# Hjinhan/Transgo

Measured on AMD Instinct MI355X. Metric: MCTS simulations/sec, higher is better.
Workload: dtype f32

## Files before the change

### include/transgo_hip.h

```cpp
#ifndef TRANSGO_HIP_H_
#define TRANSGO_HIP_H_

#include <stdbool.h>
#include <stddef.h>
#include <stdint.h>

#ifdef __cplusplus
extern "C" {
#endif

typedef struct tg_ctx tg_ctx;

typedef enum tg_status {
    TG_OK = 0,
    TG_ERR_ARG = -1,
    TG_ERR_HIP = -2,
    TG_ERR_NO_DEVICE = -3,
    TG_ERR_ARENA = -4,
    TG_ERR_STATE = -5
} tg_status;

typedef struct tg_config {
    int32_t board_size;
    int32_t encode_dim;
// ... 65 lines not shown
int tg_sp_rng_get(tg_ctx* ctx, tg_mt19937* out );
int tg_sp_rng_set(tg_ctx* ctx, const tg_mt19937* in , const uint8_t* mask );
int tg_sp_play(tg_ctx* ctx, const int32_t* actions , uint8_t* done );
int tg_sp_game_errors(tg_ctx* ctx, int32_t* n_errors, int32_t* err );
int tg_sp_tree_truncations(tg_ctx* ctx, uint64_t* blocks);

int tg_sp_pool_stats(tg_ctx* ctx, uint64_t* pool_slots, uint64_t* high_water_slots, uint64_t* in_use_slots, uint64_t* exhausted);

int tg_sp_finished(tg_ctx* ctx, int32_t* n_games, int32_t* n_positions);
int tg_sp_harvest(tg_ctx* ctx, uint32_t* obs_bits, int32_t* counts, float* z, int8_t* own, uint8_t* player, int device_out,
                  int32_t* slot, int32_t* n_moves, int32_t* winner, float* score, int8_t* terr);
int tg_sp_final(tg_ctx* ctx, float* score , float* terr , int32_t* winner );
int tg_sp_stats(tg_ctx* ctx, uint64_t* sims, uint64_t* evals, uint64_t* depth_sum, uint64_t* tie_draws, int32_t* errors,
                int32_t* max_slots);

size_t tg_net_blob_floats(int board_size, int encode_dim, int filters, int blocks);
int tg_net_load(tg_ctx* ctx, const float* blob, size_t n_floats, int rows_cap);
size_t tg_net_blob_floats_arch(int board_size, int encode_dim, int filters, const char* arch);
int tg_net_load_arch(tg_ctx* ctx, const char* arch, const float* blob, size_t n_floats, int rows_cap);
int tg_net_load_async(tg_ctx* ctx, const char* arch, const float* blob, size_t n_floats);
int tg_net_load_async_dev(tg_ctx* ctx, const char* arch, const float* d_blob , size_t n_floats);
int tg_net_load_poll(tg_ctx* ctx, int wait, int* pending);
int tg_net_predict(tg_ctx* ctx, const float* obs, int n_rows, float* policy, float* value, float* own);
int tg_net_range(tg_ctx* ctx, uint64_t* fp16_overflows, float* weight_absmax);
int tg_prof_enable(tg_ctx* ctx, int on, int max_launches);
int tg_prof_read(tg_ctx* ctx, double* conv_ms, int64_t* conv_launches, double* conv_flops);
int tg_prof_skipped(tg_ctx* ctx, int64_t* launches);
int tg_prof_enable_tree(tg_ctx* ctx, int on, int max_waves);
int tg_prof_read_tree(tg_ctx* ctx, double* collect_ms, double* absorb_ms, int64_t* waves, uint64_t* children_scored);

typedef struct tg_replay tg_replay;
int tg_replay_create(tg_ctx* ctx, int capacity_positions, tg_replay** out);
void tg_replay_destroy(tg_replay* rp);
int tg_replay_append(tg_replay* rp, const uint32_t* obs_bits , const int32_t* counts ,
                     const float* z , const int8_t* own , int n);
int tg_replay_append_dev(tg_replay* rp, const uint32_t* obs_bits, const int32_t* counts, const float* z, const int8_t* own, int n);
int tg_replay_info(const tg_replay* rp, long long* entries, long long* index, int* full);
int tg_replay_sample(tg_replay* rp, const long long* entry , int B, float* state , float* pi ,
                     float* z , float* own , int device_out);


void tg_host_mt_seed(tg_mt19937* s, uint32_t seed);
uint32_t tg_host_mt_next32(tg_mt19937* s);
double tg_host_mt_random_sample(tg_mt19937* s);
int32_t tg_host_mt_choice_index(tg_mt19937* s, int32_t k);
int tg_host_mt_dirichlet(tg_mt19937* s, double alpha, int32_t n, double* out);
// ... 26 lines not shown
```

### transgo_amd/_lib.py

```python
import ctypes
import os

_HERE = os.path.dirname(os.path.abspath(__file__))
LIB_PATH = os.path.join(_HERE, "libtransgo_hip.so")


class TgConfig(ctypes.Structure):
    _fields_ = [("board_size", ctypes.c_int32), ("encode_dim", ctypes.c_int32), ("max_step", ctypes.c_int32),
                ("komi", ctypes.c_float), ("n_games", ctypes.c_int32), ("num_simulation", ctypes.c_int32),
                ("parallel_readouts", ctypes.c_int32), ("wu_loss", ctypes.c_int32), ("c_puct1", ctypes.c_double),
                ("c_puct2", ctypes.c_double), ("arena_slots", ctypes.c_int32), ("net_blocks", ctypes.c_int32),
                ("net_filters", ctypes.c_int32), ("device", ctypes.c_int32), ("net_precision", ctypes.c_int32),
                ("record_games", ctypes.c_int32), ("pool_slots", ctypes.c_int32), ("reserved", ctypes.c_int32 * 5)]


class TgMt19937(ctypes.Structure):
    _fields_ = [("key", ctypes.c_uint32 * 624), ("pos", ctypes.c_int32)]


class TransgoError(RuntimeError):
    pass


_lib = None
# ... 25 lines not shown
    "tg_sp_search": (ctypes.c_int, [_vp, ctypes.POINTER(ctypes.c_int32)]),
    "tg_sp_root_info": (ctypes.c_int, [_vp, _vp, _vp, _vp, _vp, _vp]),
    "tg_sp_draw_uniform": (ctypes.c_int, [_vp, _vp, _vp]),
    "tg_sp_rng_state": (ctypes.c_int, [_vp, ctypes.c_int, ctypes.POINTER(TgMt19937)]),
    "tg_sp_rng_get": (ctypes.c_int, [_vp, _vp]),
    "tg_sp_rng_set": (ctypes.c_int, [_vp, _vp, _vp]),
    "tg_sp_play": (ctypes.c_int, [_vp, _vp, _vp]),
    "tg_sp_final": (ctypes.c_int, [_vp, _vp, _vp, _vp]),
    "tg_sp_game_errors": (ctypes.c_int, [_vp, ctypes.POINTER(ctypes.c_int32), _vp]),
    "tg_sp_tree_truncations": (ctypes.c_int, [_vp, ctypes.POINTER(ctypes.c_uint64)]),
    "tg_sp_pool_stats": (ctypes.c_int, [_vp] + [ctypes.POINTER(ctypes.c_uint64)] * 4),
    "tg_sp_finished": (ctypes.c_int, [_vp, ctypes.POINTER(ctypes.c_int32), ctypes.POINTER(ctypes.c_int32)]),
    "tg_sp_harvest": (ctypes.c_int, [_vp, _vp, _vp, _vp, _vp, _vp, ctypes.c_int, _vp, _vp, _vp, _vp, _vp]),
    "tg_sp_stats": (ctypes.c_int, [_vp] + [ctypes.POINTER(ctypes.c_uint64)] * 4 + [ctypes.POINTER(ctypes.c_int32)] * 2),
    "tg_net_blob_floats": (ctypes.c_size_t, [ctypes.c_int] * 4),
    "tg_net_load": (ctypes.c_int, [_vp, _vp, ctypes.c_size_t, ctypes.c_int]),
    "tg_net_blob_floats_arch": (ctypes.c_size_t, [ctypes.c_int] * 3 + [ctypes.c_char_p]),
    "tg_net_load_arch": (ctypes.c_int, [_vp, ctypes.c_char_p, _vp, ctypes.c_size_t, ctypes.c_int]),
    "tg_net_load_async": (ctypes.c_int, [_vp, ctypes.c_char_p, _vp, ctypes.c_size_t]),
    "tg_net_load_async_dev": (ctypes.c_int, [_vp, ctypes.c_char_p, _vp, ctypes.c_size_t]),
    "tg_net_load_poll": (ctypes.c_int, [_vp, ctypes.c_int, ctypes.POINTER(ctypes.c_int)]),
    "tg_net_predict": (ctypes.c_int, [_vp, _vp, ctypes.c_int, _vp, _vp, _vp]),
    "tg_net_range": (ctypes.c_int, [_vp, ctypes.POINTER(ctypes.c_uint64), ctypes.POINTER(ctypes.c_float)]),
    "tg_prof_enable": (ctypes.c_int, [_vp, ctypes.c_int, ctypes.c_int]),
    "tg_prof_read": (ctypes.c_int, [_vp, ctypes.POINTER(ctypes.c_double), ctypes.POINTER(ctypes.c_int64), ctypes.POINTER(ctypes.c_double)]),
    "tg_prof_skipped": (ctypes.c_int, [_vp, ctypes.POINTER(ctypes.c_int64)]),
    "tg_prof_enable_tree": (ctypes.c_int, [_vp, ctypes.c_int, ctypes.c_int]),
    "tg_prof_read_tree": (ctypes.c_int, [_vp, ctypes.POINTER(ctypes.c_double), ctypes.POINTER(ctypes.c_double), ctypes.POINTER(ctypes.c_int64),
                                          ctypes.POINTER(ctypes.c_uint64)]),
    "tg_replay_create": (ctypes.c_int, [_vp, ctypes.c_int, ctypes.POINTER(ctypes.c_void_p)]),
    "tg_replay_destroy": (None, [_vp]),
    "tg_replay_append": (ctypes.c_int, [_vp, _vp, _vp, _vp, _vp, ctypes.c_int]),
    "tg_replay_append_dev": (ctypes.c_int, [_vp, _vp, _vp, _vp, _vp, ctypes.c_int]),
    "tg_replay_info": (ctypes.c_int, [_vp, ctypes.POINTER(ctypes.c_longlong), ctypes.POINTER(ctypes.c_longlong), ctypes.POINTER(ctypes.c_int)]),
    "tg_replay_sample": (ctypes.c_int, [_vp, _vp, ctypes.c_int, _vp, _vp, _vp, _vp, ctypes.c_int]),
    "tg_host_mt_seed": (None, [ctypes.POINTER(TgMt19937), ctypes.c_uint32]),
    "tg_host_mt_next32": (ctypes.c_uint32, [ctypes.POINTER(TgMt19937)]),
    "tg_host_mt_random_sample": (ctypes.c_double, [ctypes.POINTER(TgMt19937)]),
    "tg_host_mt_choice_index": (ctypes.c_int32, [ctypes.POINTER(TgMt19937), ctypes.c_int32]),
    "tg_host_sub_encode": (None, [ctypes.c_int, _vp, _vp, ctypes.c_int, ctypes.c_int, ctypes.c_int]),
    "tg_host_mt_dirichlet": (ctypes.c_int, [ctypes.POINTER(TgMt19937), ctypes.c_double, ctypes.c_int32, _vp]),
}


def load():
    global _lib
# ... 57 lines not shown
```

### transgo_amd/csrc/net.hip

```cpp
#include <cmath>
#include <cstdlib>
#include <cstring>
#include <string>
#include <vector>

#include "conv_rows.h"
#include "engine.h"

using namespace tg;

namespace tg {

struct ConvW { const float* w; const float* b; };
struct BlockW { const float* s1; const float* t1; ConvW c1; ConvW c2; const float* g1; const float* g2;
                const _Float16* h1; const _Float16* h2; };
struct AttW { ConvW qkv; const float* gamma; const float* s; const float* t;
              const _Float16* x3w = nullptr; const float* x3sc = nullptr; };
struct Layer { int kind; int ridx; AttW a; };

enum Chain { CHAIN_F32 = 0, CHAIN_DMA, CHAIN_F16, CHAIN_SPLIT };
struct NetPath {
    Chain chain = CHAIN_F32;
    bool r16 = false;
    bool att_x3 = false;
    bool att_h = false;
    bool head_x2 = false;
    size_t att_lds = 0;
};

struct Net {
    int F = 0, NB = 0, C = 0, S = 0, P = 0, A = 0;
    float* blob = nullptr; size_t blob_floats = 0;
    float* wstage = nullptr;
    ConvW stem; std::vector<BlockW> blocks; std::vector<Layer> layers; const float* s_end = nullptr; const float* t_end = nullptr;
    bool pol_att = false; AttW patt; ConvW head_a; std::string arch;
    float* bufQ = nullptr; float* hca = nullptr;
    float* bufAct = nullptr;
    int prec = 0;
    const float* head_g = nullptr; const float* head_ag = nullptr;
    const _Float16* head_x2 = nullptr; const float* head_x2sc = nullptr;
    float* wsc = nullptr;
    _Float16* stem_h = nullptr; _Float16* head_h = nullptr; _Float16* x0h = nullptr;
    _Float16* wh = nullptr; _Float16* act16 = nullptr; _Float16* h16 = nullptr;
    NetPath path;
    ConvW head; const float* w_vo = nullptr; const float* b_vo = nullptr; const float* w_v = nullptr; const float* b_v = nullptr;
    const float* w_o = nullptr; const float* b_o = nullptr; const float* w_a = nullptr; const float* b_a = nullptr;
    const uint32_t* in_bits = nullptr; const int32_t* in_slot = nullptr; int in_words = 0;
    float* x0 = nullptr;
    float* bufA = nullptr; float* bufB = nullptr; float* bufH = nullptr;
    float* hc = nullptr;
// ... 32 lines not shown
        const size_t m = i >> 4;
        const int p = (int)(m % P);
        const size_t r = m / P;
        x0[i] = c < C ? obs[(r * C + c) * P + p] : 0.f;
    }
}


template <int S>
__global__ __launch_bounds__(256) void k_bits_to_rows(const uint32_t* __restrict__ bits, const int32_t* __restrict__ row_slot,
                                                      float* __restrict__ x0, int rows, int C, int W) {
    constexpr int P = S * S;
    const size_t total = (size_t)rows * P * 16;
    for (size_t i = (size_t)blockIdx.x * 256 + threadIdx.x; i < total; i += (size_t)gridDim.x * 256) {
        const int c = (int)(i & 15);
        const size_t m = i >> 4;
        const int p = (int)(m % P), k = c * P + p;
        const size_t r = m / P;
        x0[i] = c < C ? (float)((bits[(size_t)row_slot[r] * W + (k >> 5)] >> (k & 31)) & 1u) : 0.f;
    }
}

__device__ __forceinline__ size_t f32_sm_index(int srow, int c, int Msm) { return ((size_t)(c >> 4) * Msm + srow) * 16 + (c & 15); }

template <int COUT, int CT, int NPT, int EPI, bool SM = false, bool SM2 = false>
__device__ __forceinline__ void conv_epilogue(f32x4 (&acc)[CT][NPT], const int (&mrow)[NPT], int M, int co_base, int kq,
                                              float* __restrict__ out, const float* __restrict__ res, float* __restrict__ out2,
                                              const float* par, const int (&srow)[NPT], int Msm) {
    constexpr int CH = CT % 4 == 0 ? 4 : CT % 3 == 0 ? 3 : CT % 2 == 0 ? 2 : 1;
    constexpr int NCH = (CT / CH) * NPT;
    static_assert(CT % CH == 0, "chunking");
    f32x4 r[2][CH];
    auto load_res = [&](int c, f32x4* dst) {
        const int t = c / (CT / CH), h = c % (CT / CH);
        if (mrow[t] < M) {
#pragma unroll
            for (int i = 0; i < CH; ++i)
                dst[i] = *reinterpret_cast<const f32x4*>(res + (size_t)mrow[t] * COUT + co_base + (h * CH + i) * 16 + kq * 4);
        }
    };
    if (EPI == 1) load_res(0, r[0]);
#pragma unroll
    for (int c = 0; c < NCH; ++c) {
        const int t = c / (CT / CH), h = c % (CT / CH);
        if (EPI == 1 && c + 1 < NCH) load_res(c + 1, r[(c + 1) & 1]);
        if (mrow[t] < M) {
#pragma unroll
            for (int i = 0; i < CH; ++i) {
                const int ct = h * CH + i;
                const int col = ct * 16 + kq * 4;
                f32x4 v = acc[ct][t] + *reinterpret_cast<const f32x4*>(par + col);
                if (EPI == 0) {
#pragma unroll
                    for (int e = 0; e < 4; ++e) v[e] = v[e] > 0.f ? v[e] : 0.f;
                } else if (EPI == 1) {
                    v = v + r[c & 1][i];
                }
                *reinterpret_cast<f32x4*>(out + (SM ? f32_sm_index(srow[t], co_base + col, Msm) : (size_t)mrow[t] * COUT + co_base + col)) = v;
                if (out2) {
                    const f32x4 sc = *reinterpret_cast<const f32x4*>(par + COUT + col);
                    const f32x4 sh = *reinterpret_cast<const f32x4*>(par + 2 * COUT + col);
                    f32x4 u;
#pragma unroll
                    for (int e = 0; e < 4; ++e) { float w = v[e] * sc[e] + sh[e]; u[e] = w > 0.f ? w : 0.f; }
                    *reinterpret_cast<f32x4*>(out2 + (SM2 ? f32_sm_index(srow[t], co_base + col, Msm) : (size_t)mrow[t] * COUT + co_base + col)) = u;
                }
            }
        }
    }
}

template <int S, int CIN, int COUT, bool PRO, int EPI, int NTAP = 9, int NPT = 2, bool SM2 = false>
__global__ __launch_bounds__(256, (NPT > 2 ? 2 : 1)) void k_conv3x3(const float* __restrict__ in, float* __restrict__ out,
                                                 const float* __restrict__ res, const float* __restrict__ Wt,
                                                 const float* __restrict__ bias, const float* __restrict__ ps,
                                                 const float* __restrict__ pt, int M, float* __restrict__ out2 = nullptr,
                                                 const float* __restrict__ s2 = nullptr, const float* __restrict__ t2 = nullptr) {
    constexpr int P = S * S, HALO = NTAP == 9 ? S + 1 : 0;
    constexpr int TM = 64 * NPT;
    constexpr int CC = CIN < 32 ? CIN : 32;
    constexpr int RS = CC + 4;
    constexpr int NROW = TM + 2 * HALO;
    constexpr int CT = COUT / 16;
    constexpr int C4 = CC / 4;
    __shared__ float xs[NROW * RS];
    __shared__ __attribute__((aligned(16))) float par[3 * COUT];
    for (int i = tid0(); i < COUT; i += 256) { par[i] = bias[i]; par[COUT + i] = out2 ? s2[i] : 0.f; par[2 * COUT + i] = out2 ? t2[i] : 0.f; }
    constexpr bool WALL = COUT <= 16 && NTAP == 9;
    constexpr int WT = WALL ? NTAP : 1;
    __shared__ float ws[WT * COUT * RS];
    const int tid = threadIdx.x, wave = tid >> 6, lane = tid & 63;
    const int j = lane & 15, kq = lane >> 4;
    const int m0 = blockIdx.x * TM;

    unsigned vmask[NPT];
// ... 88 lines not shown
                f32x4 b[NPT];
#pragma unroll
                for (int t = 0; t < NPT; ++t) {
                    const int r = (wave * NPT + t) * 16 + j + HALO + toff;
                    b[t] = *reinterpret_cast<const f32x4*>(&xs[r * RS + sub * 16 + kq * 4]);
                    if (!((vmask[t] >> tap) & 1)) b[t] = f32x4{0.f, 0.f, 0.f, 0.f};
                }
#pragma unroll
                for (int ct = 0; ct < CT; ++ct) {
                    const f32x4 a = *reinterpret_cast<const f32x4*>(&ws[((WALL ? tap * COUT : 0) + ct * 16 + j) * RS + sub * 16 + kq * 4]);
#pragma unroll
                    for (int s = 0; s < 4; ++s)
#pragma unroll
                        for (int t = 0; t < NPT; ++t)
                            acc[ct][t] = __builtin_amdgcn_mfma_f32_16x16x4f32(a[s], b[t][s], acc[ct][t], 0, 0, 0);
                }
            }
        }
    }
    int mrow[NPT], srow[NPT];
#pragma unroll
    for (int t = 0; t < NPT; ++t) {
        mrow[t] = m0 + (wave * NPT + t) * 16 + j;
        srow[t] = SM2 ? conv_sg_row(mrow[t] / P, mrow[t] % P, P) : mrow[t];
    }
    conv_epilogue<COUT, CT, NPT, EPI, false, SM2>(acc, mrow, M, 0, kq, out, res, out2, par, srow, conv_sg_rows(M / P, P));
}

typedef __attribute__((address_space(3))) void tg_lds_void;
#define TG_VMCNT(N) asm volatile("s_waitcnt vmcnt(%0)" ::"n"(N) : "memory")
#define TG_BARRIER() do { asm volatile("" ::: "memory"); __builtin_amdgcn_s_barrier(); asm volatile("" ::: "memory"); } while (0)

using u32x4 = __attribute__((ext_vector_type(4))) unsigned int;
__device__ __forceinline__ u32x4 tg_rsrc(const void* base, unsigned bytes) {
    const unsigned long long a = (unsigned long long)base;
    return u32x4{(unsigned)a, (unsigned)(a >> 32) & 0xffffu, bytes, 0x00020000u};
}
__device__ __forceinline__ void tg_dma_global(const void* sbase , int voff_bytes, tg_lds_void* lds) {
    const unsigned la = __builtin_amdgcn_readfirstlane((unsigned)(unsigned long long)lds);
    asm volatile("s_mov_b32 m0, %0\n\ts_nop 0\n\tglobal_load_lds_dwordx4 %1, %2" ::"s"(la), "v"(voff_bytes), "s"(sbase) : "memory");
}
__device__ __forceinline__ void tg_dma_buffer(u32x4 rsrc, int voff_bytes, tg_lds_void* lds) {
    const unsigned la = __builtin_amdgcn_readfirstlane((unsigned)(unsigned long long)lds);
    asm volatile("s_mov_b32 m0, %0\n\ts_nop 0\n\tbuffer_load_dwordx4 %1, %2, 0 offen lds" ::"s"(la), "v"(voff_bytes), "s"(rsrc) : "memory");
}

__device__ __forceinline__ int swz64(int row) { return ((row >> 2) & 1) << 1; }

template <int S, int F, int EPI>
__global__ __launch_bounds__(256, (F == 128 ? 4 : 2)) void k_conv3x3_sg(const float* __restrict__ in, float* __restrict__ out,
                                                                       const float* __restrict__ res, const float* __restrict__ Ws,
                                                                       const float* __restrict__ bias, float* __restrict__ out2,
                                                                       const float* __restrict__ s2, const float* __restrict__ t2, int rows) {
    constexpr int P = S * S, CT = F / 16, CC = 16;
    constexpr int NPT = 2, TB = 64 * NPT;
    constexpr int WPW = CT / 4;
    constexpr int NSL = F / CC, D = 4;
    static_assert((F == 128 || F == 256) && NSL % 2 == 0, "tile geometry");
    __shared__ __attribute__((aligned(16))) float ws[D][F * CC];
    __shared__ __attribute__((aligned(16))) float par[3 * F];
    const int tid = threadIdx.x, lane = tid & 63;
    const int wave = __builtin_amdgcn_readfirstlane(tid >> 6);
    const int j = lane & 15, kq = lane >> 4;
    const int tpx = ((int)gridDim.x + 7) >> 3;
    const int bid = ((int)blockIdx.x & 7) * tpx + ((int)blockIdx.x >> 3);
    const int nrange = (rows + TB - 1) / TB;
    if (bid >= nrange * P) return;
    const int range = bid / P;
    const int p = conv_pos_of(bid - range * P, S);
    const int M = rows * P, Msm = conv_sg_rows(rows, P);
    for (int i = tid; i < F; i += 256) { par[i] = bias[i]; par[F + i] = out2 ? s2[i] : 0.f; par[2 * F + i] = out2 ? t2[i] : 0.f; }

    const unsigned mask = conv_tap_mask(p, S);
    const int nt = conv_tap_count(mask), nst = NSL * nt;
    const unsigned long long taps = conv_tap_list(mask);
    const int inv = nt == 9 ? 7282 : nt == 6 ? 10923 : 16384;
    auto stage = [&](int k, int* sl, int* tap) {
        *sl = (k * inv) >> 16;
        *tap = (int)(taps >> (4 * (k - *sl * nt))) & 15;
    };

    const __amdgpu_buffer_rsrc_t rin = __builtin_amdgcn_make_buffer_rsrc(const_cast<float*>(in), 0, Msm * F * 4, 0x00020000);
    const int prow = lane >> 2, pchunk = (lane & 3) ^ swz64(lane >> 2);
    auto dma_w = [&](int k) {
        int sl, tap;
        stage(k, &sl, &tap);
        const float* src = Ws + (size_t)(sl * 9 + tap) * (F * CC);
#pragma unroll
        for (int i = 0; i < WPW; ++i) {
            const int pc = wave * WPW + i;
            tg_dma_global(src + pc * 16 * CC, (prow * CC + pchunk * 4) * 4, (tg_lds_void*)(&ws[k & (D - 1)][pc * 256]));
        }
    };
    const int aoff = j * CC + ((kq ^ swz64(j)) << 2);
    const int grp0 = (range * 4 + wave) * NPT;
    const bool active = grp0 * 16 < rows;
    const int boff = ((conv_sg_row(grp0 * 16 + j, p, P)) * CC + kq * 4) * 4;
    f32x4 acc[CT][NPT], b_cur[NPT], b_next[NPT];
    auto load_b = [&](f32x4* b, int k) {
        int sl, tap;
        stage(k, &sl, &tap);
        const int ty = (tap * 11) >> 5;
        const int soff = (sl * Msm + ((ty - 1) * S + (tap - 3 * ty - 1)) * 16) * (CC * 4);
#pragma unroll
        for (int t = 0; t < NPT; ++t)
            b[t] = __builtin_bit_cast(f32x4, __builtin_amdgcn_raw_buffer_load_b128(rin, (int)((unsigned)boff + (unsigned)soff + (unsigned)(t * (P * 16 * CC * 4))), 0, 0));
    };
#pragma unroll
    for (int k = 0; k < D; ++k) dma_w(k);
    if (active) {
#pragma unroll
        for (int t = 0; t < NPT; ++t) {
            const int b = (grp0 + t) * 16 + j;
            const int m = b < rows ? b * P + p : M - 1;
#pragma unroll
            for (int ct = 0; ct < CT; ++ct) {
                acc[ct][t] = f32x4{0.f, 0.f, 0.f, 0.f};
                if (EPI == 1) acc[ct][t] = *reinterpret_cast<const f32x4*>(res + (size_t)m * F + ct * 16 + kq * 4);
            }
        }
        load_b(b_cur, 0);
        TG_VMCNT((EPI == 1 ? CT * NPT : 0) + NPT);
    } else {
        TG_VMCNT(0);
    }
    asm volatile("s_waitcnt lgkmcnt(0)" ::: "memory");
    TG_BARRIER();

#pragma unroll 1
    for (int k0 = 0; k0 < nst; k0 += 2) {
#pragma unroll
        for (int h = 0; h < 2; ++h) {
            const int k = k0 + h;
            if (active) {
                const float* wcur = ws[k & (D - 1)];
                if (k + 1 < nst) load_b(b_next, k + 1);
                __builtin_amdgcn_sched_barrier(0);
                f32x4 a_cur = *reinterpret_cast<const f32x4*>(wcur + aoff);
#pragma unroll
                for (int ct = 0; ct < CT; ++ct) {
                    f32x4 a_next = a_cur;
                    if (ct + 1 < CT) a_next = *reinterpret_cast<const f32x4*>(wcur + (ct + 1) * 256 + aoff);
#pragma unroll
                    for (int s4 = 0; s4 < 4; ++s4)
#pragma unroll
                        for (int t = 0; t < NPT; ++t)
                            acc[ct][t] = __builtin_amdgcn_mfma_f32_16x16x4f32(a_cur[s4], b_cur[t][s4], acc[ct][t], 0, 0, 0);
                    a_cur = a_next;
                }
#pragma unroll
                for (int t = 0; t < NPT; ++t) b_cur[t] = b_next[t];
            }
            TG_VMCNT(0);
        }
        TG_BARRIER();
        if (k0 + 4 < nst) { dma_w(k0 + 4); dma_w(k0 + 5); }
    }
    if (!active) return;
    int mrow[NPT], srow[NPT];
#pragma unroll
    for (int t = 0; t < NPT; ++t) {
        const int b = (grp0 + t) * 16 + j;
        mrow[t] = b < rows ? b * P + p : M;
        srow[t] = conv_sg_row(b, p, P);
    }
    conv_epilogue<F, CT, NPT, (EPI == 1 ? 2 : EPI), EPI == 0, true>(acc, mrow, M, 0, kq, out, res, out2, par, srow, Msm);
}

__device__ __forceinline__ size_t h16_index(int m, int c, int M) { return (((size_t)(c >> 5) * 4 + ((c >> 3) & 3)) * M + m) * 8 + (c & 7); }

template <int N>
__device__ __forceinline__ void vmcnt_uniform(int n) {
    if (n >= N) TG_VMCNT(N);
    else if constexpr (N > 0) vmcnt_uniform<N - 1>(n);
}

__device__ __forceinline__ int x2_index(int c) { return ((c >> 4) << 5) + (c & 15); }
template <int F, int CT, int NPT, int EPI, bool R16, bool X2 = false>
__device__ __forceinline__ void conv_epilogue_h8(f32x4 (&acc)[CT][NPT], const int (&mrow)[NPT], int M, int co_base, int kq,
                                                 float* __restrict__ out32, _Float16* __restrict__ out16, const float* par, int pstride,
                                                 float wsc, float& amax) {
    static_assert(CT % 2 == 0, "tile pairs");
    static_assert(!(X2 && R16), "split precision keeps the f32 residual stream");
#pragma unroll
    for (int t = 0; t < NPT; ++t) {
        if (mrow[t] >= M) continue;
#pragma unroll
        for (int u = 0; u < CT / 2; ++u) {
            const int lc = u * 32 + kq * 8, col = co_base + lc;
// ... 1167 lines not shown
    const int grid_h = (M + 255) / 256;
    constexpr int COS = F / 128;
    const int nblk_h2 = COS == 1 ? grid_h : (grid_h + 7) / 8 * 8 * COS;
    const double conv_flops = 2.0 * 9.0 * (double)F * (double)F * (double)M;
    constexpr int WQ = F / 4 + F / 4 + F;
    const bool big = (long long)M * F * 4 >= (1ll << 31);
    Chain chain = n->path.chain;
    if (chain == CHAIN_DMA && (long long)conv_sg_rows(rows, P) * F * 4 >= (1ll << 31)) chain = CHAIN_F32;
    if (chain == CHAIN_SPLIT && big) TG_FAIL(ctx, TG_ERR_ARG, "split-precision path: rows * P * F * 4 bytes must stay below 2 GiB per activation buffer");
    if (chain == CHAIN_F16 && (long long)M * F * 2 >= (1ll << 31)) TG_FAIL(ctx, TG_ERR_ARG, "fp16 path: rows * P * F * 2 bytes must stay below 2 GiB per activation buffer");
    const bool h16 = chain == CHAIN_F16 || chain == CHAIN_SPLIT, x2 = chain == CHAIN_SPLIT;
    const bool head16 = chain == CHAIN_F16 || (x2 && n->path.head_x2);
    auto wsc = [&](size_t conv) { return x2 ? n->wsc + conv : nullptr; };
    const size_t nl = n->layers.size(), nb = n->blocks.size();
    auto next_bn = [&](size_t j, const float** sn, const float** tn) -> bool {
        *sn = nullptr; *tn = nullptr;
        if (chain == CHAIN_F32) return false;
        if (j < nl && n->layers[j].kind == 0) { const BlockW& b = n->blocks[n->layers[j].ridx]; *sn = b.s1; *tn = b.t1; return true; }
        if (j == nl && head16) { *sn = n->s_end; *tn = n->t_end; return true; }
        return false;
    };

    float* x = n->bufA; float* y = n->bufB;
    auto stem = [&](bool act, const float* sn, const float* tn) {
        if constexpr (WIDE) {
            if (h16) {
                auto* k = x2 ? &k_conv3x3_h2<S, 64, F, 4, false, true> : n->path.r16 ? &k_conv3x3_h2<S, 64, F, 4, true> : &k_conv3x3_h2<S, 64, F, 4>;
                hipLaunchKernelGGL(k, dim3(nblk_h2), dim3(256), 0, st, n->x0h, x, act ? n->act16 : nullptr, nullptr, n->stem_h, n->stem.b,
                                   sn, tn, M, nblk_h2, wsc(2 * nb), n->range);
                return;
            }
            if (chain == CHAIN_DMA) {
                hipLaunchKernelGGL((k_conv3x3<S, 16, F, false, 0, 9, 2, true>), dim3(grid), dim3(256), 0, st, n->x0, x, nullptr, n->stem.w,
                                   n->stem.b, nullptr, nullptr, M, act ? n->bufAct : nullptr, sn, tn);
                return;
            }
        }
        hipLaunchKernelGGL((k_conv3x3<S, 16, F, false, 0>), dim3(grid), dim3(256), 0, st, n->x0, x, nullptr, n->stem.w, n->stem.b, nullptr, nullptr, M);
    };
    auto block = [&](const BlockW& b, int ridx, float* out, bool act, const float* sn, const float* tn) {
        if constexpr (WIDE) {
            if (h16) {
                auto* k1 = x2 ? &k_conv3x3_h2<S, 2 * F, F, 0, false, true> : &k_conv3x3_h2<S, F, F, 0>;
                auto* k2 = x2 ? &k_conv3x3_h2<S, 2 * F, F, 1, false, true> : n->path.r16 ? &k_conv3x3_h2<S, F, F, 1, true> : &k_conv3x3_h2<S, F, F, 1>;
                { ProfScope ps(n, st, conv_flops);
                  hipLaunchKernelGGL(k1, dim3(nblk_h2), dim3(256), 0, st, n->act16, nullptr, n->h16, nullptr, b.h1, b.c1.b, nullptr, nullptr,
                                     M, nblk_h2, wsc(2 * ridx), n->range); }
                { ProfScope ps(n, st, conv_flops);
                  hipLaunchKernelGGL(k2, dim3(nblk_h2), dim3(256), 0, st, n->h16, out, act ? n->act16 : nullptr, x, b.h2, b.c2.b, sn, tn,
                                     M, nblk_h2, wsc(2 * ridx + 1), n->range); }
                return;
            }
            if (chain == CHAIN_DMA) {
                const int grid_sd = ((rows + 127) / 128 * P + 7) / 8 * 8;
                auto* k1 = &k_conv3x3_sg<S, F, 0>;
                auto* k2 = &k_conv3x3_sg<S, F, 1>;
                { ProfScope ps(n, st, conv_flops);
                  hipLaunchKernelGGL(k1, dim3(grid_sd), dim3(256), 0, st, n->bufAct, n->bufH, nullptr, b.g1, b.c1.b, nullptr, nullptr, nullptr, rows); }
                { ProfScope ps(n, st, conv_flops);
                  hipLaunchKernelGGL(k2, dim3(grid_sd), dim3(256), 0, st, n->bufH, out, x, b.g2, b.c2.b, act ? n->bufAct : nullptr, sn, tn, rows); }
                return;
            }
        }
        { ProfScope ps(n, st, conv_flops);
          hipLaunchKernelGGL((k_conv3x3<S, F, F, true, 0, 9, NPT>), dim3(grid_f), dim3(256), 0, st, x, n->bufH, nullptr, b.c1.w, b.c1.b, b.s1, b.t1, M); }
        { ProfScope ps(n, st, conv_flops);
          hipLaunchKernelGGL((k_conv3x3<S, F, F, false, 1, 9, NPT>), dim3(grid_f), dim3(256), 0, st, n->bufH, out, x, b.c2.w, b.c2.b, nullptr, nullptr, M); }
    };
    auto attention = [&](const AttW& a, const float* xin, float* xout, const float* ps, const float* pt, bool act, const float* sn, const float* tn) -> int {
        if constexpr (S == 9 && F == 128) {
            if (x2) {
                constexpr int lds3 = (int)(sizeof(_Float16) * F / 16 * WQ * 32 + sizeof(float) * (WQ + 6 * F) + 4096);
                const int nwg = (rows + 3) / 4 < 256 ? (rows + 3) / 4 : 256;
                auto* k = ps ? &k_attention_x3<S, F, true> : &k_attention_x3<S, F, false>;
                hipLaunchKernelGGL(k, dim3(nwg), dim3(256), lds3, st, xin, xout, act ? n->act16 : nullptr, a.x3w, a.qkv.b, a.x3sc,
                                   a.gamma, a.s, a.t, ps, pt, sn, tn, rows, n->range);
                return 0;
            }
            if (chain == CHAIN_F16 && n->path.att_h) {
                constexpr int ldsh = (int)(sizeof(_Float16) * F / 32 * WQ * 32 + sizeof(float) * (WQ + 6 * F) + 4096);
                const int nwg = (rows + 3) / 4 < 256 ? (rows + 3) / 4 : 256;
                auto* k = ps ? &k_attention_h<S, F, true> : &k_attention_h<S, F, false>;
                hipLaunchKernelGGL(k, dim3(nwg), dim3(256), ldsh, st, xin, xout, act ? n->act16 : nullptr, a.x3w, a.qkv.b,
// ... 33 lines not shown
    auto head_conv = [&](const float* in, float* outp, const float* Wg, const ConvW& cw, const float* ps, const float* pt) {
        const char* hg = getenv("TG_HEAD_GEMM");
        if (hg && atoi(hg) == 0) {
            auto* k = ps ? &k_conv3x3<S, F, 16, true, 0> : &k_conv3x3<S, F, 16, false, 0>;
            hipLaunchKernelGGL(k, dim3(grid), dim3(256), 0, st, in, outp, nullptr, cw.w, cw.b, ps, pt, M, nullptr, nullptr, nullptr);
            return;
        }
        constexpr int TMH = 64 * (S == 9 ? 3 : 4) - 2 * (S + 1);
        const int nt = (M + TMH - 1) / TMH, g = nt < 512 ? nt : 512;
        auto* k = ps ? &k_head_gemm<S, F, true> : &k_head_gemm<S, F, false>;
        hipLaunchKernelGGL(k, dim3(g), dim3(256), 0, st, in, outp, Wg, cw.b, ps, pt, M, nt);
    };

    if (h16) {
        int g0h = (int)(((size_t)M * 8 + 255) / 256); if (g0h > 65535) g0h = 65535;
        if (n->in_bits) hipLaunchKernelGGL((k_bits_to_rows_h<S>), dim3(g0h), dim3(256), 0, st, n->in_bits, n->in_slot, n->x0h, rows, n->C, n->in_words);
        else hipLaunchKernelGGL((k_obs_to_rows_h<S>), dim3(g0h), dim3(256), 0, st, obs, n->x0h, rows, n->C);
    } else {
        int g0 = (int)(((size_t)M * 16 + 255) / 256); if (g0 > 65535) g0 = 65535;
        if (n->in_bits) hipLaunchKernelGGL((k_bits_to_rows<S>), dim3(g0), dim3(256), 0, st, n->in_bits, n->in_slot, n->x0, rows, n->C, n->in_words);
        else hipLaunchKernelGGL((k_obs_to_rows<S>), dim3(g0), dim3(256), 0, st, obs, n->x0, rows, n->C);
    }
    const float* sn; const float* tn;
    { const bool act = next_bn(0, &sn, &tn); stem(act, sn, tn); }
    for (size_t i = 0; i < nl; ++i) {
        const Layer& L = n->layers[i];
        const bool act = next_bn(i + 1, &sn, &tn);
        if (L.kind == 1) {
            if (attention(L.a, x, y, nullptr, nullptr, act, sn, tn)) TG_FAIL(ctx, TG_ERR_ARG, "attention blocks: no kernel for this shape and precision (built: f32 at 9x9 with 32 / 64 / 128 / 256 filters and at 19x19 with 128 / 256, f16 at 9x9 with 128, f32x3 at 9x9 with 128 / 256)");
        } else {
            block(n->blocks[L.ridx], L.ridx, i + 1 == nl && head16 && !n->pol_att ? nullptr : y, act, sn, tn);
        }
        float* t = x; x = y; y = t;
    }
    if (!head16) {
        head_conv(x, n->hc, n->head_g, n->head, n->s_end, n->t_end);
    } else if constexpr (WIDE) {
        if (!x2) {
            hipLaunchKernelGGL((k_head_h<S, F>), dim3(grid_h), dim3(256), 0, st, n->act16, n->hc, n->head_h, n->head.b, M);
        } else if constexpr (F == 128) {
            constexpr int TMH = 64 * (S == 9 ? 3 : 4) - 2 * (S + 1);
            const int nt = (M + TMH - 1) / TMH, g = nt < 512 ? nt : 512;
            hipLaunchKernelGGL((k_head_gemm_x2<S, F>), dim3(g), dim3(256), 0, st, n->act16, n->hc, n->head_x2, n->head_x2sc, n->head.b, M, nt);
        }
    }
    const float* hca = n->hc;
    if (n->pol_att) {
        if (attention(n->patt, x, y, n->s_end, n->t_end, false, nullptr, nullptr)) TG_FAIL(ctx, TG_ERR_ARG, "attention policy head: no kernel for this shape and precision (built: f32 at 9x9 with 32 / 64 / 128 / 256 filters and at 19x19 with 128 / 256, f16 at 9x9 with 128, f32x3 at 9x9 with 128 / 256)");
        head_conv(y, n->hca, n->head_ag, n->head_a, nullptr, nullptr);
        hca = n->hca;
    }
    hipLaunchKernelGGL((k_heads<S>), dim3((rows + HeadRows<S>::N - 1) / HeadRows<S>::N), dim3(256), 0, st, n->hc, hca, n->w_vo, n->b_vo, n->w_v, n->b_v,
                       n->w_o, n->b_o, n->w_a, n->b_a, policy, value, own, rows);
    TG_HIP(ctx, hipGetLastError());
// ... 152 lines not shown
    return TG_OK;
}

int adopt_pending(tg_ctx* ctx, Net* n, bool wait) {
    if (!n->pending) return TG_OK;
    if (wait) TG_HIP(ctx, hipEventSynchronize(n->loaded));
    else if (hipEventQuery(n->loaded) != hipSuccess) return TG_OK;
    n->active ^= 1;
    bind_weights(n, n->active);
    n->pending = false;
    TG_HIP(ctx, hipEventRecord(n->swapped, ctx->stream));
    return TG_OK;
}

NetPath net_path(int S, int F, int prec, const std::string& trunk, bool pol) {
    const size_t P = (size_t)S * S, Wq = (size_t)F / 4 * 2 + F;
    const bool any_att = pol || trunk.find('A') != std::string::npos;
    NetPath p;
    if (prec == 3) p.chain = CHAIN_SPLIT;
    else if (prec >= 1) p.chain = CHAIN_F16;
    else if (F == 128 || F == 256) {
        const char* dma = getenv("TG_DMA_CONV");
        p.chain = dma && atoi(dma) == 0 ? CHAIN_F32 : CHAIN_DMA;
    }
    p.r16 = prec == 2;
    p.att_x3 = prec == 3 && any_att && F == 128 && S == 9;
    p.att_h = prec == 1 && any_att && F == 128 && S == 9;
    p.head_x2 = prec == 3 && F == 128 && !trunk.empty() && trunk.back() == 'R';
    const size_t lds = sizeof(float) * (P * Wq + P * (P + 1));
    p.att_lds = any_att && lds <= 160 * 1024 ? lds : 0;
    return p;
}

}

extern "C" {

size_t tg_net_blob_floats(int board_size, int encode_dim, int filters, int blocks) {
    return expected_floats(board_size, encode_dim, filters, std::string((size_t)(blocks > 0 ? blocks : 0), 'R'));
}

size_t tg_net_blob_floats_arch(int board_size, int encode_dim, int filters, const char* arch) {
    return arch ? expected_floats(board_size, encode_dim, filters, arch) : 0;
}

int tg_net_load(tg_ctx* ctx, const float* blob, size_t n_floats, int rows_cap) {
// ... 15 lines not shown
    if (!ctx->eng) { ctx->eng = new Engine(); }
    Engine* e = ctx->eng;
    if (rows_cap <= 0) rows_cap = e->rows_cap > 0 ? e->rows_cap : 256;
    if (e->rows_cap > rows_cap) rows_cap = e->rows_cap;
    Net* n = e->net;
    const int prec = ctx->cfg.net_precision;
    if (prec < 0 || prec > 3) TG_FAIL(ctx, TG_ERR_ARG, "net_precision: 0 (f32), 1 (fp16 storage, f32 accumulate, f32 residual stream), 2 (fp16 residual stream too) or 3 (split precision: fp16 hi + lo operands, f32 accumulate)");
    if (n && (n->rows_cap < rows_cap || n->arch != arch || n->prec != prec)) { tg_net_destroy(ctx); n = nullptr; }
    const size_t P = (size_t)S * S, A = P + 1, Wq = (size_t)F / 4 * 2 + F;
    const bool any_att = pol || trunk.find('A') != std::string::npos;
    int NB = 0; for (char c : trunk) NB += c == 'R';
    if (prec >= 1 && ((any_att && !(prec == 3 && S == 9) && !(prec == 1 && S == 9 && F == 128)) || (F != 128 && F != 256)))
        TG_FAIL(ctx, TG_ERR_ARG, "net_precision 1 / 2 (fp16 matrix cores) is built for towers with 128 or 256 filters; attention layers are built for 1 (fp16 storage, f32 residual stream) at 9x9 with 128 filters and for 3 (split precision) at 9x9, not for 2, nor for 1 at 19x19 or with 256 filters");
    if (prec == 0 && any_att && S == 19 && F != 128 && F != 256)
        TG_FAIL(ctx, TG_ERR_ARG, "attention layers at 19x19 are built for net_precision 0 (f32) with 128 or 256 filters (k_attention_t); at 9x9 for every filter count of the f32 path");
    if (!n) {
        n = new Net();
        e->net = n;
        n->S = S; n->P = (int)P; n->A = (int)A; n->C = C; n->F = F; n->NB = NB; n->rows_cap = rows_cap; n->arch = arch; n->pol_att = pol;
        n->blob_floats = n_floats; n->prec = prec;
        const NetPath& p = n->path = net_path(S, F, prec, trunk, pol);
        const bool h16 = p.chain == CHAIN_F16 || p.chain == CHAIN_SPLIT, x2 = p.chain == CHAIN_SPLIT;
        const size_t act = sizeof(float) * (size_t)rows_cap * P * F;
        TG_HIP(ctx, hipMalloc((void**)&n->bufA, act));
        TG_HIP(ctx, hipMalloc((void**)&n->bufB, act));
        const size_t act_sm = sizeof(float) * (size_t)conv_sg_rows(rows_cap, (int)P) * F;
        TG_HIP(ctx, hipMalloc((void**)&n->bufH, act_sm));
        TG_HIP(ctx, hipMalloc((void**)&n->x0, sizeof(float) * (size_t)rows_cap * P * 16));
        TG_HIP(ctx, hipMalloc((void**)&n->hc, sizeof(float) * (size_t)rows_cap * P * 16));
        TG_HIP(ctx, hipMalloc((void**)&n->own, sizeof(float) * (size_t)rows_cap * P));
        TG_HIP(ctx, hipMalloc((void**)&n->range, sizeof(unsigned) * 4));
        TG_HIP(ctx, hipMemset(n->range, 0, sizeof(unsigned) * 4));

        if (any_att && !p.att_h) TG_HIP(ctx, hipMalloc((void**)&n->bufQ, sizeof(float) * (size_t)rows_cap * P * Wq));
        if (pol) TG_HIP(ctx, hipMalloc((void**)&n->hca, sizeof(float) * (size_t)rows_cap * P * 16));
        const size_t wcopy = (size_t)(NB > 0 ? 2 * NB : 1) * 9 * F * F;
        if (p.chain == CHAIN_DMA) TG_HIP(ctx, hipMalloc((void**)&n->bufAct, act_sm));
        for (Net::WeightSet& w : n->sets) {
            TG_HIP(ctx, hipMalloc((void**)&w.blob, sizeof(float) * n_floats));
            TG_HIP(ctx, hipMalloc((void**)&w.head_g, sizeof(float) * 64 * (size_t)F));
            if (pol) TG_HIP(ctx, hipMalloc((void**)&w.head_ag, sizeof(float) * 64 * (size_t)F));
            if (p.chain == CHAIN_DMA) TG_HIP(ctx, hipMalloc((void**)&w.wstage, sizeof(float) * wcopy));
            if (h16) {
                TG_HIP(ctx, hipMalloc((void**)&w.wh, sizeof(_Float16) * wcopy * (x2 ? 2 : 1)));
                TG_HIP(ctx, hipMalloc((void**)&w.stem_h, sizeof(_Float16) * 9 * (size_t)F * 64));
            }
            if (p.chain == CHAIN_F16) TG_HIP(ctx, hipMalloc((void**)&w.head_h, sizeof(_Float16) * 9 * 16 * (size_t)F));
            if (x2) TG_HIP(ctx, hipMalloc((void**)&w.wsc, sizeof(float) * 2 * (size_t)(2 * NB + 1)));
            if (p.head_x2) {
                TG_HIP(ctx, hipMalloc((void**)&w.head_x2, sizeof(_Float16) * 64 * (size_t)F * 2));
                TG_HIP(ctx, hipMalloc((void**)&w.head_x2sc, sizeof(float) * 2));
            }
            if (p.att_x3) {
                size_t n_att = pol ? 1 : 0; for (char c : trunk) n_att += c == 'A';
                TG_HIP(ctx, hipMalloc((void**)&w.att_h, sizeof(_Float16) * n_att * ((size_t)F / 16 * Wq * 32)));
                TG_HIP(ctx, hipMalloc((void**)&w.att_sc, sizeof(float) * 2 * n_att));
            }
            if (p.att_h) {
                size_t n_att = pol ? 1 : 0; for (char c : trunk) n_att += c == 'A';
                TG_HIP(ctx, hipMalloc((void**)&w.att_h, sizeof(_Float16) * n_att * ((size_t)F / 32 * Wq * 32)));
// ... 128 lines not shown
    Net* n = ctx->eng->net;
    { int rc = adopt_pending(ctx, n, false); if (rc) return rc; }
    const size_t P = n->P, A = n->A, C = n->C;
    int done = 0;
    tg::DevBuf& din = ctx->env_f32; tg::DevBuf& dout = ctx->env_in;
    while (done < n_rows) {
        const int k = (n_rows - done) < n->rows_cap ? (n_rows - done) : n->rows_cap;
        if (din.reserve(sizeof(float) * k * C * P) || dout.reserve(sizeof(float) * k * (A + 1)))
            TG_FAIL(ctx, TG_ERR_HIP, "hipMalloc failed (predict scratch)");
        float* d_pol = (float*)dout.p; float* d_val = d_pol + (size_t)k * A;
        TG_HIP(ctx, hipMemcpyAsync(din.p, obs + (size_t)done * C * P, sizeof(float) * k * C * P, hipMemcpyHostToDevice, ctx->stream));
        int rc = forward(ctx, n, (const float*)din.p, k, d_pol, d_val, own ? n->own : nullptr);
        if (rc) return rc;
        TG_HIP(ctx, hipMemcpyAsync(policy + (size_t)done * A, d_pol, sizeof(float) * k * A, hipMemcpyDeviceToHost, ctx->stream));
        TG_HIP(ctx, hipMemcpyAsync(value + done, d_val, sizeof(float) * k, hipMemcpyDeviceToHost, ctx->stream));
        if (own) TG_HIP(ctx, hipMemcpyAsync(own + (size_t)done * P, n->own, sizeof(float) * k * P, hipMemcpyDeviceToHost, ctx->stream));
        TG_HIP(ctx, hipStreamSynchronize(ctx->stream));
        done += k;
    }
    return TG_OK;
}


int tg_net_range(tg_ctx* ctx, uint64_t* fp16_overflows, float* weight_absmax) {
    if (!ctx || !ctx->eng || !ctx->eng->net) return TG_ERR_STATE;
    Net* n = ctx->eng->net;
    TG_HIP(ctx, hipSetDevice(ctx->cfg.device));
    unsigned host[4] = {0, 0, 0, 0};
    TG_HIP(ctx, hipStreamSynchronize(ctx->stream));
    TG_HIP(ctx, hipMemcpy(host, n->range, sizeof(host), hipMemcpyDeviceToHost));
    if (fp16_overflows) *fp16_overflows = host[0];
    if (weight_absmax) { float f; memcpy(&f, &host[1 + n->active], sizeof(f)); *weight_absmax = f; }
    if (host[0])
        ctx->err = "fp16 overflow: " + std::to_string(host[0]) + " epilogue tiles rounded a value beyond +-65504 to fp16 (net_precision " +
                   std::to_string(n->prec) + "); outputs since then may be inf/NaN -- use net_precision 0 for these weights";
    return TG_OK;
}

int tg_prof_enable(tg_ctx* ctx, int on, int max_launches) {
    if (!ctx || !ctx->eng || !ctx->eng->net) return TG_ERR_STATE;
    Net* n = ctx->eng->net;
    TG_HIP(ctx, hipSetDevice(ctx->cfg.device));
    if (on) {
        const size_t want = 2 * (size_t)(max_launches > 0 ? max_launches : 4096);
        while (n->ev.size() < want) { hipEvent_t ev; TG_HIP(ctx, hipEventCreate(&ev)); n->ev.push_back(ev); }
        n->ev_used = 0; n->conv_ms = 0; n->conv_launches = 0; n->conv_flops = 0; n->conv_skipped = 0;
// ... 28 lines not shown
```

Baseline: 533,900.

## Fuse pre-activation BN-ReLU into conv loads and keep trunk activations in shared-group layout

In the DMA conv chain, residual blocks can now apply the BN+ReLU pre-activation while loading the input operand (one_stream mode, on by default). This removes the separate activated copy (bufAct) that the previous conv epilogue wrote and the next conv read. Residual and output tensors stay in the sg layout, and the buffers are sized to match. An env var selects the mode, and a query API reports the layout. The cost is extra VALU work for the BN+ReLU inside the MFMA loop, which is repeated for every tap.

```diff
diff --git a/include/transgo_hip.h b/include/transgo_hip.h
--- a/include/transgo_hip.h
+++ b/include/transgo_hip.h
@@ -111,6 +111,7 @@
 int tg_net_load_async_dev(tg_ctx* ctx, const char* arch, const float* d_blob , size_t n_floats);
 int tg_net_load_poll(tg_ctx* ctx, int wait, int* pending);
 int tg_net_predict(tg_ctx* ctx, const float* obs, int n_rows, float* policy, float* value, float* own);
+int tg_net_stream_layout(tg_ctx* ctx, int* one_stream, int* act_copy);
 int tg_net_range(tg_ctx* ctx, uint64_t* fp16_overflows, float* weight_absmax);
 int tg_prof_enable(tg_ctx* ctx, int on, int max_launches);
 int tg_prof_read(tg_ctx* ctx, double* conv_ms, int64_t* conv_launches, double* conv_flops);
diff --git a/transgo_amd/_lib.py b/transgo_amd/_lib.py
--- a/transgo_amd/_lib.py
+++ b/transgo_amd/_lib.py
@@ -71,6 +71,7 @@
     "tg_net_load_poll": (ctypes.c_int, [_vp, ctypes.c_int, ctypes.POINTER(ctypes.c_int)]),
     "tg_net_predict": (ctypes.c_int, [_vp, _vp, ctypes.c_int, _vp, _vp, _vp]),
     "tg_net_range": (ctypes.c_int, [_vp, ctypes.POINTER(ctypes.c_uint64), ctypes.POINTER(ctypes.c_float)]),
+    "tg_net_stream_layout": (ctypes.c_int, [_vp, ctypes.POINTER(ctypes.c_int), ctypes.POINTER(ctypes.c_int)]),
     "tg_prof_enable": (ctypes.c_int, [_vp, ctypes.c_int, ctypes.c_int]),
     "tg_prof_read": (ctypes.c_int, [_vp, ctypes.POINTER(ctypes.c_double), ctypes.POINTER(ctypes.c_int64), ctypes.POINTER(ctypes.c_double)]),
     "tg_prof_skipped": (ctypes.c_int, [_vp, ctypes.POINTER(ctypes.c_int64)]),
diff --git a/transgo_amd/csrc/net.hip b/transgo_amd/csrc/net.hip
--- a/transgo_amd/csrc/net.hip
+++ b/transgo_amd/csrc/net.hip
@@ -26,6 +26,7 @@
     bool att_h = false;
     bool head_x2 = false;
     size_t att_lds = 0;
+    int one_stream = 0;
 };
 
 struct Net {
@@ -104,6 +105,13 @@
 }
 
 __device__ __forceinline__ size_t f32_sm_index(int srow, int c, int Msm) { return ((size_t)(c >> 4) * Msm + srow) * 16 + (c & 15); }
+__device__ __forceinline__ float bn_relu(float v, float s, float t) { const float w = v * s + t; return w > 0.f ? w : 0.f; }
+__device__ __forceinline__ float bn_relu_unpacked(float v, float s, float t) {
+    float w;
+    asm("v_mul_f32 %0, %1, %2" : "=v"(w) : "v"(v), "v"(s));
+    asm("v_add_f32 %0, %1, %2" : "=v"(w) : "v"(w), "v"(t));
+    return w > 0.f ? w : 0.f;
+}
 
 template <int COUT, int CT, int NPT, int EPI, bool SM = false, bool SM2 = false>
 __device__ __forceinline__ void conv_epilogue(f32x4 (&acc)[CT][NPT], const int (&mrow)[NPT], int M, int co_base, int kq,
@@ -144,7 +152,7 @@
                     const f32x4 sh = *reinterpret_cast<const f32x4*>(par + 2 * COUT + col);
                     f32x4 u;
 #pragma unroll
-                    for (int e = 0; e < 4; ++e) { float w = v[e] * sc[e] + sh[e]; u[e] = w > 0.f ? w : 0.f; }
+                    for (int e = 0; e < 4; ++e) u[e] = bn_relu(v[e], sc[e], sh[e]);
                     *reinterpret_cast<f32x4*>(out2 + (SM2 ? f32_sm_index(srow[t], co_base + col, Msm) : (size_t)mrow[t] * COUT + co_base + col)) = u;
                 }
             }
@@ -152,7 +160,7 @@
     }
 }
 
-template <int S, int CIN, int COUT, bool PRO, int EPI, int NTAP = 9, int NPT = 2, bool SM2 = false>
+template <int S, int CIN, int COUT, bool PRO, int EPI, int NTAP = 9, int NPT = 2, bool SM2 = false, bool SM1 = false>
 __global__ __launch_bounds__(256, (NPT > 2 ? 2 : 1)) void k_conv3x3(const float* __restrict__ in, float* __restrict__ out,
                                                  const float* __restrict__ res, const float* __restrict__ Wt,
                                                  const float* __restrict__ bias, const float* __restrict__ ps,
@@ -287,9 +295,9 @@
 #pragma unroll
     for (int t = 0; t < NPT; ++t) {
         mrow[t] = m0 + (wave * NPT + t) * 16 + j;
-        srow[t] = SM2 ? conv_sg_row(mrow[t] / P, mrow[t] % P, P) : mrow[t];
-    }
-    conv_epilogue<COUT, CT, NPT, EPI, false, SM2>(acc, mrow, M, 0, kq, out, res, out2, par, srow, conv_sg_rows(M / P, P));
+        srow[t] = SM2 || SM1 ? conv_sg_row(mrow[t] / P, mrow[t] % P, P) : mrow[t];
+    }
+    conv_epilogue<COUT, CT, NPT, EPI, SM1, SM2>(acc, mrow, M, 0, kq, out, res, out2, par, srow, conv_sg_rows(M / P, P));
 }
 
 typedef __attribute__((address_space(3))) void tg_lds_void;
@@ -312,7 +320,7 @@
 
 __device__ __forceinline__ int swz64(int row) { return ((row >> 2) & 1) << 1; }
 
-template <int S, int F, int EPI>
+template <int S, int F, int EPI, bool SIN = false, bool SOUT = false>
 __global__ __launch_bounds__(256, (F == 128 ? 4 : 2)) void k_conv3x3_sg(const float* __restrict__ in, float* __restrict__ out,
                                                                        const float* __restrict__ res, const float* __restrict__ Ws,
                                                                        const float* __restrict__ bias, float* __restrict__ out2,
@@ -334,7 +342,8 @@
     const int range = bid / P;
     const int p = conv_pos_of(bid - range * P, S);
     const int M = rows * P, Msm = conv_sg_rows(rows, P);
-    for (int i = tid; i < F; i += 256) { par[i] = bias[i]; par[F + i] = out2 ? s2[i] : 0.f; par[2 * F + i] = out2 ? t2[i] : 0.f; }
+    constexpr bool ACT = EPI == 0 && SIN;
+    for (int i = tid; i < F; i += 256) { par[i] = bias[i]; par[F + i] = out2 || ACT ? s2[i] : 0.f; par[2 * F + i] = out2 || ACT ? t2[i] : 0.f; }
 
     const unsigned mask = conv_tap_mask(p, S);
     const int nt = conv_tap_count(mask), nst = NSL * nt;
@@ -362,26 +371,45 @@
     const bool active = grp0 * 16 < rows;
     const int boff = ((conv_sg_row(grp0 * 16 + j, p, P)) * CC + kq * 4) * 4;
     f32x4 acc[CT][NPT], b_cur[NPT], b_next[NPT];
+    int sl_b = 0, sl_p = -1;
+    f32x4 bsc, bsh;
     auto load_b = [&](f32x4* b, int k) {
         int sl, tap;
         stage(k, &sl, &tap);
+        sl_b = sl;
         const int ty = (tap * 11) >> 5;
         const int soff = (sl * Msm + ((ty - 1) * S + (tap - 3 * ty - 1)) * 16) * (CC * 4);
 #pragma unroll
         for (int t = 0; t < NPT; ++t)
             b[t] = __builtin_bit_cast(f32x4, __builtin_amdgcn_raw_buffer_load_b128(rin, (int)((unsigned)boff + (unsigned)soff + (unsigned)(t * (P * 16 * CC * 4))), 0, 0));
     };
+    auto act_b = [&](f32x4* dst, const f32x4* b) {
+        if (sl_b != sl_p) {
+            sl_p = sl_b;
+            bsc = *reinterpret_cast<const f32x4*>(par + F + sl_b * CC + kq * 4);
+            bsh = *reinterpret_cast<const f32x4*>(par + 2 * F + sl_b * CC + kq * 4);
+        }
+#pragma unroll
+        for (int t = 0; t < NPT; ++t)
+#pragma unroll
+            for (int e = 0; e < 4; ++e) dst[t][e] = bn_relu_unpacked(b[t][e], bsc[e], bsh[e]);
+    };
 #pragma unroll
     for (int k = 0; k < D; ++k) dma_w(k);
     if (active) {
 #pragma unroll
         for (int t = 0; t < NPT; ++t) {
             const int b = (grp0 + t) * 16 + j;
-            const int m = b < rows ? b * P + p : M - 1;
+            [[maybe_unused]] const int m = b < rows ? b * P + p : M - 1;
 #pragma unroll
             for (int ct = 0; ct < CT; ++ct) {
                 acc[ct][t] = f32x4{0.f, 0.f, 0.f, 0.f};
-                if (EPI == 1) acc[ct][t] = *reinterpret_cast<const f32x4*>(res + (size_t)m * F + ct * 16 + kq * 4);
+                if constexpr (EPI == 1 && SIN) {
+                    const __amdgpu_buffer_rsrc_t rres = __builtin_amdgcn_make_buffer_rsrc(const_cast<float*>(res), 0, Msm * F * 4, 0x00020000);
+                    acc[ct][t] = __builtin_bit_cast(f32x4, __builtin_amdgcn_raw_buffer_load_b128(rres, (int)((unsigned)boff + (unsigned)(ct * Msm * (CC * 4)) + (unsigned)(t * (P * 16 * CC * 4))), 0, 0));
+                } else if constexpr (EPI == 1) {
+                    acc[ct][t] = *reinterpret_cast<const f32x4*>(res + (size_t)m * F + ct * 16 + kq * 4);
+                }
             }
         }
         load_b(b_cur, 0);
@@ -391,6 +419,13 @@
     }
     asm volatile("s_waitcnt lgkmcnt(0)" ::: "memory");
     TG_BARRIER();
+    if constexpr (ACT) {
+        if (active) act_b(b_cur, b_cur);
+        else {
+#pragma unroll
+            for (int t = 0; t < NPT; ++t) b_cur[t] = f32x4{0.f, 0.f, 0.f, 0.f};
+        }
+    }
 
 #pragma unroll 1
     for (int k0 = 0; k0 < nst; k0 += 2) {
@@ -413,8 +448,13 @@
                             acc[ct][t] = __builtin_amdgcn_mfma_f32_16x16x4f32(a_cur[s4], b_cur[t][s4], acc[ct][t], 0, 0, 0);
                     a_cur = a_next;
                 }
-#pragma unroll
-                for (int t = 0; t < NPT; ++t) b_cur[t] = b_next[t];
+                if constexpr (ACT) {
+                    __builtin_amdgcn_sched_barrier(0);
+                    act_b(b_cur, b_next);
+                } else {
+#pragma unroll
+                    for (int t = 0; t < NPT; ++t) b_cur[t] = b_next[t];
+                }
             }
             TG_VMCNT(0);
         }
@@ -429,7 +469,7 @@
         mrow[t] = b < rows ? b * P + p : M;
         srow[t] = conv_sg_row(b, p, P);
     }
-    conv_epilogue<F, CT, NPT, (EPI == 1 ? 2 : EPI), EPI == 0, true>(acc, mrow, M, 0, kq, out, res, out2, par, srow, Msm);
+    conv_epilogue<F, CT, NPT, (EPI == 1 ? 2 : EPI), EPI == 0 || SOUT, true>(acc, mrow, M, 0, kq, out, res, out2, par, srow, Msm);
 }
 
 __device__ __forceinline__ size_t h16_index(int m, int c, int M) { return (((size_t)(c >> 5) * 4 + ((c >> 3) & 3)) * M + m) * 8 + (c & 7); }
@@ -1643,7 +1683,10 @@
     };
 
     float* x = n->bufA; float* y = n->bufB;
-    auto stem = [&](bool act, const float* sn, const float* tn) {
+    const int one = chain == CHAIN_DMA ? n->path.one_stream : 0;
+    auto conv_layer = [&](size_t j) { return j < nl && n->layers[j].kind == 0; };
+    float* const act2 = one == 1 ? nullptr : n->bufAct;
+    auto stem = [&](bool act, const float* sn, const float* tn, bool sout) {
         if constexpr (WIDE) {
             if (h16) {
                 auto* k = x2 ? &k_conv3x3_h2<S, 64, F, 4, false, true> : n->path.r16 ? &k_conv3x3_h2<S, 64, F, 4, true> : &k_conv3x3_h2<S, 64, F, 4>;
@@ -1652,14 +1695,15 @@
                 return;
             }
             if (chain == CHAIN_DMA) {
-                hipLaunchKernelGGL((k_conv3x3<S, 16, F, false, 0, 9, 2, true>), dim3(grid), dim3(256), 0, st, n->x0, x, nullptr, n->stem.w,
-                                   n->stem.b, nullptr, nullptr, M, act ? n->bufAct : nullptr, sn, tn);
+                auto* k = sout ? &k_conv3x3<S, 16, F, false, 0, 9, 2, true, true> : &k_conv3x3<S, 16, F, false, 0, 9, 2, true>;
+                hipLaunchKernelGGL(k, dim3(grid), dim3(256), 0, st, n->x0, x, nullptr, n->stem.w,
+                                   n->stem.b, nullptr, nullptr, M, act ? act2 : nullptr, sn, tn);
                 return;
             }
         }
         hipLaunchKernelGGL((k_conv3x3<S, 16, F, false, 0>), dim3(grid), dim3(256), 0, st, n->x0, x, nullptr, n->stem.w, n->stem.b, nullptr, nullptr, M);
     };
-    auto block = [&](const BlockW& b, int ridx, float* out, bool act, const float* sn, const float* tn) {
+    auto block = [&](const BlockW& b, int ridx, float* out, bool act, const float* sn, const float* tn, bool sin, bool sout) {
         if constexpr (WIDE) {
             if (h16) {
                 auto* k1 = x2 ? &k_conv3x3_h2<S, 2 * F, F, 0, false, true> : &k_conv3x3_h2<S, F, F, 0>;
@@ -1674,12 +1718,15 @@
             }
             if (chain == CHAIN_DMA) {
                 const int grid_sd = ((rows + 127) / 128 * P + 7) / 8 * 8;
-                auto* k1 = &k_conv3x3_sg<S, F, 0>;
-                auto* k2 = &k_conv3x3_sg<S, F, 1>;
+                const bool onload = sin && one == 1;
+                auto* k1 = onload ? &k_conv3x3_sg<S, F, 0, true> : &k_conv3x3_sg<S, F, 0>;
+                auto* k2 = sin ? (sout ? &k_conv3x3_sg<S, F, 1, true, true> : &k_conv3x3_sg<S, F, 1, true, false>)
+                               : (sout ? &k_conv3x3_sg<S, F, 1, false, true> : &k_conv3x3_sg<S, F, 1>);
                 { ProfScope ps(n, st, conv_flops);
-                  hipLaunchKernelGGL(k1, dim3(grid_sd), dim3(256), 0, st, n->bufAct, n->bufH, nullptr, b.g1, b.c1.b, nullptr, nullptr, nullptr, rows); }
+                  hipLaunchKernelGGL(k1, dim3(grid_sd), dim3(256), 0, st, onload ? x : n->bufAct, n->bufH, nullptr, b.g1, b.c1.b, nullptr,
+                                     onload ? b.s1 : nullptr, onload ? b.t1 : nullptr, rows); }
                 { ProfScope ps(n, st, conv_flops);
-                  hipLaunchKernelGGL(k2, dim3(grid_sd), dim3(256), 0, st, n->bufH, out, x, b.g2, b.c2.b, act ? n->bufAct : nullptr, sn, tn, rows); }
+                  hipLaunchKernelGGL(k2, dim3(grid_sd), dim3(256), 0, st, n->bufH, out, x, b.g2, b.c2.b, act ? act2 : nullptr, sn, tn, rows); }
                 return;
             }
         }
@@ -1759,14 +1806,17 @@
         else hipLaunchKernelGGL((k_obs_to_rows<S>), dim3(g0), dim3(256), 0, st, obs, n->x0, rows, n->C);
     }
     const float* sn; const float* tn;
-    { const bool act = next_bn(0, &sn, &tn); stem(act, sn, tn); }
+    bool sm = one && conv_layer(0);
+    { const bool act = next_bn(0, &sn, &tn); stem(act, sn, tn, sm); }
     for (size_t i = 0; i < nl; ++i) {
         const Layer& L = n->layers[i];
         const bool act = next_bn(i + 1, &sn, &tn);
+        const bool sin = sm;
+        sm = one && L.kind == 0 && conv_layer(i + 1);
         if (L.kind == 1) {
             if (attention(L.a, x, y, nullptr, nullptr, act, sn, tn)) TG_FAIL(ctx, TG_ERR_ARG, "attention blocks: no kernel for this shape and precision (built: f32 at 9x9 with 32 / 64 / 128 / 256 filters and at 19x19 with 128 / 256, f16 at 9x9 with 128, f32x3 at 9x9 with 128 / 256)");
         } else {
-            block(n->blocks[L.ridx], L.ridx, i + 1 == nl && head16 && !n->pol_att ? nullptr : y, act, sn, tn);
+            block(n->blocks[L.ridx], L.ridx, i + 1 == nl && head16 && !n->pol_att ? nullptr : y, act, sn, tn, sin, sm);
         }
         float* t = x; x = y; y = t;
     }
@@ -1965,6 +2015,8 @@
     else if (F == 128 || F == 256) {
         const char* dma = getenv("TG_DMA_CONV");
         p.chain = dma && atoi(dma) == 0 ? CHAIN_F32 : CHAIN_DMA;
+        const char* one = getenv("TG_ONE_STREAM");
+        p.one_stream = one && one[0] >= '0' && one[0] <= '2' && !one[1] ? one[0] - '0' : 1;
     }
     p.r16 = prec == 2;
     p.att_x3 = prec == 3 && any_att && F == 128 && S == 9;
@@ -2026,9 +2078,9 @@
         const NetPath& p = n->path = net_path(S, F, prec, trunk, pol);
         const bool h16 = p.chain == CHAIN_F16 || p.chain == CHAIN_SPLIT, x2 = p.chain == CHAIN_SPLIT;
         const size_t act = sizeof(float) * (size_t)rows_cap * P * F;
-        TG_HIP(ctx, hipMalloc((void**)&n->bufA, act));
-        TG_HIP(ctx, hipMalloc((void**)&n->bufB, act));
         const size_t act_sm = sizeof(float) * (size_t)conv_sg_rows(rows_cap, (int)P) * F;
+        TG_HIP(ctx, hipMalloc((void**)&n->bufA, p.chain == CHAIN_DMA ? act_sm : act));
+        TG_HIP(ctx, hipMalloc((void**)&n->bufB, p.chain == CHAIN_DMA ? act_sm : act));
         TG_HIP(ctx, hipMalloc((void**)&n->bufH, act_sm));
         TG_HIP(ctx, hipMalloc((void**)&n->x0, sizeof(float) * (size_t)rows_cap * P * 16));
         TG_HIP(ctx, hipMalloc((void**)&n->hc, sizeof(float) * (size_t)rows_cap * P * 16));
@@ -2039,7 +2091,7 @@
         if (any_att && !p.att_h) TG_HIP(ctx, hipMalloc((void**)&n->bufQ, sizeof(float) * (size_t)rows_cap * P * Wq));
         if (pol) TG_HIP(ctx, hipMalloc((void**)&n->hca, sizeof(float) * (size_t)rows_cap * P * 16));
         const size_t wcopy = (size_t)(NB > 0 ? 2 * NB : 1) * 9 * F * F;
-        if (p.chain == CHAIN_DMA) TG_HIP(ctx, hipMalloc((void**)&n->bufAct, act_sm));
+        if (p.chain == CHAIN_DMA && (p.one_stream != 1 || trunk.find("AR") != std::string::npos)) TG_HIP(ctx, hipMalloc((void**)&n->bufAct, act_sm));
         for (Net::WeightSet& w : n->sets) {
             TG_HIP(ctx, hipMalloc((void**)&w.blob, sizeof(float) * n_floats));
             TG_HIP(ctx, hipMalloc((void**)&w.head_g, sizeof(float) * 64 * (size_t)F));
@@ -2214,6 +2266,14 @@
 }
 
 
+int tg_net_stream_layout(tg_ctx* ctx, int* one_stream, int* act_copy) {
+    if (!ctx || !ctx->eng || !ctx->eng->net) return TG_ERR_STATE;
+    const Net* n = ctx->eng->net;
+    if (one_stream) *one_stream = n->path.chain == CHAIN_DMA ? n->path.one_stream : 0;
+    if (act_copy) *act_copy = n->bufAct != nullptr;
+    return TG_OK;
+}
+
 int tg_net_range(tg_ctx* ctx, uint64_t* fp16_overflows, float* weight_absmax) {
     if (!ctx || !ctx->eng || !ctx->eng->net) return TG_ERR_STATE;
     Net* n = ctx->eng->net;
```

Result: faster. 543,200, median of 6 (+1.8%).
